# rbrito/deprecated-lame-mirror

Hardware: AMD Instinct MI355X
Metric: encoded audio seconds/sec (x real-time) at 44.1kHz stereo CBR128 (higher is better)
Workload: dtype f32

## Files before the change

### deprecated-lame-mirror_amd/csrc/lh_analysis.hip

```cpp
#include <stdint.h>
#include <math.h>

#ifdef LH_EMU
#include "hipemu.h"
#define LH_CONST static const
#else
#include <hip/hip_runtime.h>
#define LH_CONST __device__ static const
#endif

#if defined(LH_APROF) && !defined(LH_EMU)
__shared__ unsigned long long *lh_ap_base;
#define LH_PT(var) unsigned long long var = clock64()
#define LH_PA(idx, var) do { if (c.lane == 0) atomicAdd(&lh_ap_base[LH_NPROF * c.wave + 20 + (idx)], clock64() - var); } while (0)
#define LH_PC(idx) do { } while (0)
#endif
#define LH_CUSTOM_LDS "lh_lds_analysis.h"
#define LH_CUSTOM_SMP
#define LH_FZ_X(i) ((((i) >> 4) & 2) | (((i) >> 3) & 24) | (((i) >> 5) & 4))
#define LH_FZ(i) ((i) ^ LH_FZ_X(i))
#define LH_STAGE_IDX(i) LH_FZ(i)
#include "lh_static_tables.h"
#include "lh_dev_common.h"
#if !defined(LH_EMU)
#define LH_KRESTRICT __restrict__
#else
#define LH_KRESTRICT
#endif

#define LH_SPAN (lh_lds.work)
LH_DEVFN float
lh_smp(const LhCtx & c, int ch, int i)
{
    return LH_SPAN[ch * LH_BLKSIZE + LH_FZ(i)];
}

#include "lh_dev_psy_core.h"

struct LhGranuleAt {
    int     live;
    int     gr;
    long long at;
    long long frame_base;
};

LH_DEVFN LhGranuleAt
lh_granule_at(const LhStreamDesc & d, int g)
{
    LhGranuleAt o;
    int const nf = d.frame_end - d.frame_begin;
    int const fr = g / LH_NGR;
    o.live = g < LH_NGR * nf;
    o.gr = g - fr * LH_NGR;
    o.at = d.out_index + d.mid_rel + fr;
    o.frame_base = (long long) (576 * LH_NGR) * (d.frame_begin + fr) - LH_MF_START;
    return o;
}

LH_DEVFN LhStreamDesc
lh_desc_uniform(const LhStreamDesc * descs, int sidx)
{
    LhStreamDesc d = descs[sidx];
    d.pcm_l = lh_uni_ll(d.pcm_l);
    d.pcm_r = lh_uni_ll(d.pcm_r);
    d.pcm_base = lh_uni_ll(d.pcm_base);
    d.nsamples = lh_uni_ll(d.nsamples);
    d.out_index = lh_uni_ll(d.out_index);
    d.mid_rel = lh_uni_i(d.mid_rel);
    d.frame_begin = lh_uni_i(d.frame_begin);
    d.frame_end = lh_uni_i(d.frame_end);
    return d;
}

#ifdef LH_LSF
#define lh_attack_kernel lh_attack_kernel_lsf
#define lh_attack_scan_kernel lh_attack_scan_kernel_lsf
#define lh_analysis_kernel lh_analysis_kernel_lsf
#define lh_launch_analysis lh_launch_analysis_lsf
#define lh_emu_analysis lh_emu_analysis_lsf
#endif

#if defined(LH_APROF) && !defined(LH_EMU)
#define LH_AP_T0() unsigned long long ap_t = clock64()
#define LH_AP(k) do { unsigned long long const n_ = clock64(); if (c.lane == 0) atomicAdd(&aprof[64 * 0 + LH_NPROF * c.wave + (k)], n_ - ap_t); ap_t = n_; } while (0)
#else
#define LH_AP_T0() do { } while (0)
#define LH_AP(k) do { } while (0)
#endif
#define LH_FIR_SPAN 640

#ifndef LH_EMU
extern "C" __global__ void __launch_bounds__(64)
#else
void
#endif
lh_attack_kernel(const LhConfig * LH_KRESTRICT cfg, const int16_t * LH_KRESTRICT pcm, const float *pcmf, const LhStreamDesc * descs, LhMidFrame * frames,
                 int nstreams)
{
    __shared__ float span[2 * LH_FIR_SPAN];
    int const sidx = (int) blockIdx.y;
    LhCtx   c;
    c.cfg = cfg;
    c.T = nullptr;
    c.st = nullptr;
    c.pcm = pcm;
    c.pcmf = pcmf;
    c.d = lh_desc_uniform(descs, sidx);
    c.tid = (int) threadIdx.x;
    c.lane = c.tid;
    c.wave = 0;
    LhGranuleAt const ga = lh_granule_at(c.d, (int) blockIdx.x);
    if (!ga.live)
        return;
    int const lane = c.lane;
    int const n_chn_psy = (cfg->mode == LH_MODE_JOINT_STEREO) ? 4 : cfg->channels;
    int const bufbase = 576 + ga.gr * 576 - LH_FFTOFFSET;
    int const firbase = bufbase + 576 - 350 - LH_NSFIRLEN + 192;
    LhMidGr *mg = &frames[ga.at].small.gr[ga.gr];
    lh_stage_span < LH_FIR_SPAN, 64, 1 > (c, span, span + LH_FIR_SPAN, ga.frame_base + firbase);
    LH_WAVE_SYNC();
    {
        int const i0 = 9 * lane;
        float   x[2][30], y[2][9];
#pragma unroll
        for (int ch = 0; ch < 2; ch++)
#pragma unroll
            for (int t = 0; t < 30; t++)
                x[ch][t] = span[ch * LH_FIR_SPAN + i0 + t];
#pragma unroll
        for (int ch = 0; ch < 2; ch++)
#pragma unroll
            for (int m = 0; m < 9; m++) {
                float   sum1 = x[ch][m + 10], sum2 = 0.0;
#pragma unroll
                for (int j = 0; j < ((LH_NSFIRLEN - 1) / 2) - 1; j += 2) {
                    sum1 += lh_hp_fir[j] * (x[ch][m + j] + x[ch][m + LH_NSFIRLEN - j]);
                    sum2 += lh_hp_fir[j + 1] * (x[ch][m + j + 1] + x[ch][m + LH_NSFIRLEN - j - 1]);
                }
                y[ch][m] = sum1 + sum2;
            }
        LH_WAVE_SYNC();
#pragma unroll
        for (int ch = 0; ch < 2; ch++)
#pragma unroll
            for (int m = 0; m < 9; m++)
                span[ch * LH_FIR_SPAN + i0 + m] = y[ch][m];
    }
    LH_WAVE_SYNC();
    float   fl[9], fr[9];
#pragma unroll
    for (int k = 0; k < 9; k++) {
        fl[k] = span[lane + 64 * k];
        fr[k] = span[LH_FIR_SPAN + lane + 64 * k];
    }
    for (int chn = 0; chn < n_chn_psy; chn++) {
        uint32_t pk[8], pk8 = 0;
#pragma unroll
        for (int k = 0; k < 9; k++) {
            float const l = fl[k], r = fr[k];
            float const v = (chn == 0) ? l : (chn == 1) ? r : (chn == 2) ? l + r : l - r;
            if (k < 8)
                pk[k] = lh_f32_as_u32(lh_fabsf(v));
            else
                pk8 = lh_f32_as_u32(lh_fabsf(v));
        }
        {
            uint32_t const m8 = lh_wave_max8(pk);
            uint32_t const m9 = lh_wave_max_u32(pk8);
            if (lane < 9)
                mg->peak[chn][lane] = lh_u32_as_f32(lane == 8 ? m9 : m8);
        }
    }
}

#ifndef LH_SCAN_BLOCK
#define LH_SCAN_BLOCK 4
#endif
#ifndef LH_EMU
extern "C" __global__ void __launch_bounds__(64)
#else
void
#endif
lh_attack_scan_kernel(const LhConfig * LH_KRESTRICT cfg, const LhTables * LH_KRESTRICT T, const LhStreamDesc * descs, const LhStreamState * states,
                      LhMidFrame * frames, int nstreams)
{
    int const sidx = (int) blockIdx.x;
    int const lane = (int) threadIdx.x;
    LhStreamDesc const d = lh_desc_uniform(descs, sidx);
    int const nf = d.frame_end - d.frame_begin;
    if (nf <= 0)
        return;
    const LhStreamState *st = &states[sidx];
    int const n_chn_psy = lh_uni_i((cfg->mode == LH_MODE_JOINT_STEREO) ? 4 : cfg->channels);
    int const channels = lh_uni_i(cfg->channels), short_blocks = lh_uni_i(cfg->short_blocks);
    int const chn = lane >> 4, i = lane & 15, grp = lane & 48;
    int const mine = chn < n_chn_psy;
    float   le = st->last_en_subshort[chn][i < 9 ? i : 0];
    int     last_att = st->last_attacks[chn];
    float const thresh = T->attack_threshold[chn];
    int     bt_old0 = lh_uni_i(st->blocktype_old[0]), bt_old1 = lh_uni_i(st->blocktype_old[1]);
    int const ng = LH_NGR * nf;
    float   pk_blk[LH_SCAN_BLOCK];
#pragma unroll
    for (int j = 0; j < LH_SCAN_BLOCK; j++) {
        int const g = (j < ng) ? j : 0;
        pk_blk[j] = frames[d.out_index + d.mid_rel + g / LH_NGR].small.gr[g % LH_NGR].peak[chn][i < 9 ? i : 0];
    }
    for (int g0 = 0; g0 < ng; g0 += LH_SCAN_BLOCK) {
        float   pk_cur[LH_SCAN_BLOCK], ssf_blk[LH_SCAN_BLOCK];
        int     nsa_blk[LH_SCAN_BLOCK][4];
#pragma unroll
        for (int j = 0; j < LH_SCAN_BLOCK; j++) {
            int const gn = g0 + LH_SCAN_BLOCK + j, g = (gn < ng) ? gn : 0;
            pk_cur[j] = pk_blk[j];
            pk_blk[j] = frames[d.out_index + d.mid_rel + g / LH_NGR].small.gr[g % LH_NGR].peak[chn][i < 9 ? i : 0];
        }
#pragma unroll
        for (int j = 0; j < LH_SCAN_BLOCK; j++) {
            float const pk = pk_cur[j];
            float const fresh = pk < 1.0f ? 1.0f : pk;
            float const old = lh_shfl_f32(le, grp + ((i + 6) & 15)), older = lh_shfl_f32(le, grp + ((i + 4) & 15));
            float const got = lh_shfl_f32(fresh, grp + ((i - 3) & 15));
            float const e = (i < 3) ? old : got;
            float const e1 = lh_shfl_f32(e, grp + ((i - 1) & 15)), e0 = lh_shfl_f32(e, grp + ((i - 2) & 15));
            float const then = (i < 3) ? older : e0;
            float const ai = (i < 3) ? e / then : (e > then) ? e / then : (then > e * 10.0f) ? then / (e * 10.0f) : 0.0f;
            float const whole = e0 + e1 + e;
            int const tail_low = e * 6 < whole, mid_low = e1 * 6 < whole;
            uint64_t const over_all = lh_ballot(i < 12 && ai > thresh);
            unsigned const over = (unsigned) (over_all >> (16 * chn)) & 0xfffu;
            float   en_short[4];
            en_short[0] = lh_shfl_f32(whole, grp + 2);
            en_short[1] = lh_shfl_f32(whole, grp + 5);
            en_short[2] = lh_shfl_f32(whole, grp + 8);
            en_short[3] = lh_shfl_f32(whole, grp + 11);
            ssf_blk[j] = tail_low ? (mid_low ? 0.25f : 0.5f) : 1.0f;
            int    *nsa = nsa_blk[j];
            le = fresh;
            for (int gq = 0; gq < 4; gq++) {
                unsigned const bits = (over >> (3 * gq)) & 7u;
                nsa[gq] = bits ? ((bits & 1u) ? 1 : (bits & 2u) ? 2 : 3) : 0;
            }
            for (int q = 1; q < 4; q++) {
                float const u = en_short[q - 1];
                float const v = en_short[q];
                float const m = (u > v) ? u : v;
                if (m < 40000) {
                    if (u < 1.7f * v && v < 1.7f * u) {
                        if (q == 1 && nsa[0] <= nsa[q])
                            nsa[0] = 0;
                        nsa[q] = 0;
                    }
                }
            }
        }
#pragma unroll
        for (int j = 0; j < LH_SCAN_BLOCK; j++) {
            int const g = g0 + j;
            if (g >= ng)
                break;
            int const fr = g / LH_NGR, gr = g - fr * LH_NGR;
            LhMidGr *mg = &frames[d.out_index + d.mid_rel + fr].small.gr[gr];
            int    *nsa = nsa_blk[j];
            float const ssf = ssf_blk[j];
            int     uselong = 1;
            if (nsa[0] <= last_att)
                nsa[0] = 0;
            if (last_att == 3 || nsa[0] + nsa[1] + nsa[2] + nsa[3]) {
                uselong = 0;
                if (nsa[1] && nsa[0])
                    nsa[1] = 0;
                if (nsa[2] && nsa[1])
                    nsa[2] = 0;
                if (nsa[3] && nsa[2])
                    nsa[3] = 0;
            }
            if (!mine) {
                nsa[0] = nsa[1] = nsa[2] = nsa[3] = 0;
                uselong = 1;
            }
            else
                last_att = nsa[2];
            if (i == 5 || i == 8 || i == 11)
                mg->sub_short_factor[chn][(i - 5) / 3] = mine ? ssf : 1.0f;
            if (i < 4)
                mg->ns_attacks[chn][i] = (int8_t) (i == 0 ? nsa[0] : i == 1 ? nsa[1] : i == 2 ? nsa[2] : nsa[3]);
            {
                uint64_t const shorts = lh_ballot(!uselong);
                int const s0 = (int) (shorts & 1u), s1 = (int) ((shorts >> 16) & 1u), s23 = (int) ((shorts >> 32) & 0x10001u) != 0;
                int     ul0 = !s0, ul1 = (channels == 2) ? !s1 : 1;
                int     btd[2];
                if (s23)
                    ul0 = ul1 = 0;
                if (short_blocks == 1 && !(ul0 && ul1))
                    ul0 = ul1 = 0;
                if (short_blocks == 2)
                    ul0 = ul1 = 1;
                if (short_blocks == 3)
                    ul0 = ul1 = 0;
                for (int ch = 0; ch < 2; ch++) {
                    int     blocktype = LH_NORM_TYPE;
                    int     was = ch ? bt_old1 : bt_old0;
                    if (ch ? ul1 : ul0) {
                        if (was == LH_SHORT_TYPE)
                            blocktype = LH_STOP_TYPE;
                    }
                    else {
                        blocktype = LH_SHORT_TYPE;
                        if (was == LH_NORM_TYPE)
                            was = LH_START_TYPE;
                        if (was == LH_STOP_TYPE)
                            was = LH_SHORT_TYPE;
                    }
                    btd[ch] = was;
                    if (ch)
                        bt_old1 = lh_uni_i(blocktype);
                    else
                        bt_old0 = lh_uni_i(blocktype);
                }
                if (lane < 2) {
                    mg->uselong[lane] = (int8_t) (lane ? ul1 : ul0);
                    mg->block_type[lane] = (int8_t) (lane ? btd[1] : btd[0]);
                }
            }
        }
    }
}

template < int K1 > LH_DEVFN void
lh_fht_unit_fz(lh_f32x4 tw, float *fz, int u)
{
    constexpr int kx = K1 >> 1, k2 = K1 << 1, k3 = k2 + K1, k4 = k2 << 1;
    int const blk = u / kx, i = u - blk * kx;
    int const axis = (i == 0);
    int const lo = blk * k4 + i;
    int const hi = blk * k4 + (axis ? kx : K1 - i);
    int     al[4], ah[4];
    if (K1 == 4) {
        int const x = LH_FZ_X(lo);
#pragma unroll
        for (int j = 0; j < 4; j++) {
            al[j] = (lo + j * K1) ^ x;
            ah[j] = (hi + j * K1) ^ x;
        }
    }
    else if (K1 == 16) {
        int const x = LH_FZ_X(blk * k4);
#pragma unroll
        for (int j = 0; j < 4; j++) {
            al[j] = (lo + j * K1) ^ x ^ (j >= 2 ? 2 : 0);
            ah[j] = (hi + j * K1) ^ x ^ (j >= 2 ? 2 : 0);
        }
    }
    else if (K1 == 64) {
#pragma unroll
        for (int j = 0; j < 4; j++) {
            al[j] = (lo + j * K1) ^ LH_FZ_X(64 * j);
            ah[j] = (hi + j * K1) ^ (2 ^ LH_FZ_X(64 * j));
        }
    }
    else {
        int const xl = LH_FZ_X(lo), xh = LH_FZ_X(hi);
#pragma unroll
        for (int j = 0; j < 4; j++) {
            al[j] = (lo + j * K1) ^ xl;
            ah[j] = (hi + j * K1) ^ xh;
        }
    }
    float const p0 = fz[al[0]], p1 = fz[al[1]], p2 = fz[al[2]], p3 = fz[al[3]];
    float const q0 = fz[ah[0]], q1 = fz[ah[1]], q2 = fz[ah[2]], q3 = fz[ah[3]];
    float const s01 = p0 + p1, d01 = p0 - p1, s23 = p2 + p3, d23 = p2 - p3;
    float const r2 = (float) (LH_SQRT2 * q2), r3 = (float) (LH_SQRT2 * q3);
    float const t01 = q0 + q1, u01 = q0 - q1;
    float const a_l0 = s01 + s23, a_l1 = d01 + d23, a_l2 = s01 - s23, a_l3 = d01 - d23;
    float const a_h0 = t01 + r2, a_h1 = u01 + r3, a_h2 = t01 - r2, a_h3 = u01 - r3;
    LhRot const rq1 = lh_rot(tw.z, tw.w, p1, q1);
    LhRot const rq3 = lh_rot(tw.z, tw.w, p3, q3);
    float const le = p0 + rq1.along, lm = p0 - rq1.along;
    float const he = q0 + rq1.across, hm = q0 - rq1.across;
    float const l2e = p2 + rq3.along, l2m = p2 - rq3.along;
    float const h2e = q2 + rq3.across, h2m = q2 - rq3.across;
    LhRot const ra = lh_rot(tw.x, tw.y, l2e, h2m);
    LhRot const rb = lh_rot(tw.y, tw.x, h2e, l2m);
    fz[al[0]] = axis ? a_l0 : le + ra.along;
    fz[al[1]] = axis ? a_l1 : lm + rb.across;
    fz[al[2]] = axis ? a_l2 : le - ra.along;
    fz[al[3]] = axis ? a_l3 : lm - rb.across;
    fz[ah[0]] = axis ? a_h0 : he + rb.along;
    fz[ah[1]] = axis ? a_h1 : hm + ra.across;
    fz[ah[2]] = axis ? a_h2 : he - rb.along;
    fz[ah[3]] = axis ? a_h3 : hm - ra.across;
}

LH_DEVFN void
lh_fft_long_inplace(const LhCtx & c, float *x)
{
    const float *w = c.T->fft_window;
    int const lane = c.lane;
    float   o[2][8];
#pragma unroll
    for (int q = 0; q < 2; q++) {
        int const jj = lane + 64 * q;
        int const i = (int) lh_rev8((unsigned) jj);
        const float *xs = x + (i ^ LH_FZ_X(i));
        float   f0, f1, f2, f3, ww;
        f0 = w[i] * xs[0];
        ww = w[i + 0x200] * xs[0x200];
        f1 = f0 - ww;
        f0 = f0 + ww;
        f2 = w[i + 0x100] * xs[0x100];
        ww = w[i + 0x300] * xs[0x300];
        f3 = f2 - ww;
        f2 = f2 + ww;
        o[q][0] = f0 + f2;
        o[q][2] = f0 - f2;
        o[q][1] = f1 + f3;
        o[q][3] = f1 - f3;
        f0 = w[i + 0x001] * xs[0x001];
        ww = w[i + 0x201] * xs[0x201];
        f1 = f0 - ww;
        f0 = f0 + ww;
        f2 = w[i + 0x101] * xs[0x101];
        ww = w[i + 0x301] * xs[0x301];
        f3 = f2 - ww;
        f2 = f2 + ww;
        o[q][4] = f0 + f2;
        o[q][6] = f0 - f2;
        o[q][5] = f1 + f3;
        o[q][7] = f1 - f3;
    }
    {
        lh_f32x4 tw[4][2];
#pragma unroll
        for (int stage = 0; stage < 4; stage++) {
            int const kx = 2 << (2 * stage);
#pragma unroll
            for (int q = 0; q < 2; q++)
                tw[stage][q] = *(const lh_f32x4 *) c.T->fht_tw[stage][(lane + 64 * q) % kx];
        }
        LH_WAVE_SYNC_MEM();
#pragma unroll
        for (int q = 0; q < 2; q++) {
            int const at = 4 * (lane + 64 * q), xa = LH_FZ_X(at);
#pragma unroll
            for (int k = 0; k < 4; k++) {
                x[(at + k) ^ xa] = o[q][k];
                x[(at + k + LH_BLKSIZE / 2) ^ xa] = o[q][4 + k];
            }
        }
        LH_WAVE_SYNC_MEM();
#pragma unroll
        for (int q = 0; q < 2; q++)
            lh_fht_unit_fz < 4 > (tw[0][q], x, lane + 64 * q);
        LH_WAVE_SYNC_MEM();
#pragma unroll
        for (int q = 0; q < 2; q++)
            lh_fht_unit_fz < 16 > (tw[1][q], x, lane + 64 * q);
        LH_WAVE_SYNC_MEM();
#pragma unroll
        for (int q = 0; q < 2; q++)
            lh_fht_unit_fz < 64 > (tw[2][q], x, lane + 64 * q);
        LH_WAVE_SYNC_MEM();
#pragma unroll
        for (int q = 0; q < 2; q++)
            lh_fht_unit_fz < 256 > (tw[3][q], x, lane + 64 * q);
        LH_WAVE_SYNC_MEM();
    }
}

LH_DEVFN void
lh_fft_short_inplace(const LhCtx & c, float *x)
{
    const float *ws = c.T->fft_window_s;
    int const lane = c.lane;
    float   o[2][8];
#pragma unroll
    for (int q = 0; q < 2; q++) {
        int const t = lane + 64 * q, tt = t < 3 * (LH_BLKSIZE_S / 8) ? t : 0;
        int const b = tt >> 5, j = tt & 31;
        int const k = (576 / 3) * (b + 1);
        int const i = (int) lh_rev8((unsigned) (j << 2));
        float   f0, f1, f2, f3, w;
        f0 = ws[i] * x[LH_FZ(i + k)];
        w = ws[0x7f - i] * x[LH_FZ(i + k + 0x80)];
        f1 = f0 - w;
        f0 = f0 + w;
        f2 = ws[i + 0x40] * x[LH_FZ(i + k + 0x40)];
        w = ws[0x3f - i] * x[LH_FZ(i + k + 0xc0)];
        f3 = f2 - w;
        f2 = f2 + w;
        o[q][0] = f0 + f2;
        o[q][2] = f0 - f2;
        o[q][1] = f1 + f3;
        o[q][3] = f1 - f3;
        f0 = ws[i + 0x01] * x[LH_FZ(i + k + 0x01)];
        w = ws[0x7e - i] * x[LH_FZ(i + k + 0x81)];
        f1 = f0 - w;
        f0 = f0 + w;
        f2 = ws[i + 0x41] * x[LH_FZ(i + k + 0x41)];
        w = ws[0x3e - i] * x[LH_FZ(i + k + 0xc1)];
        f3 = f2 - w;
        f2 = f2 + w;
        o[q][4] = f0 + f2;
        o[q][6] = f0 - f2;
        o[q][5] = f1 + f3;
        o[q][7] = f1 - f3;
    }
    LH_WAVE_SYNC_MEM();
#pragma unroll
    for (int q = 0; q < 2; q++) {
        int const t = lane + 64 * q;
        if (t < 3 * (LH_BLKSIZE_S / 8)) {
            int const at = (t >> 5) * LH_BLKSIZE_S + 4 * (t & 31);
#pragma unroll
            for (int k = 0; k < 4; k++) {
                x[LH_FZ(at + k)] = o[q][k];
                x[LH_FZ(at + k + LH_BLKSIZE_S / 2)] = o[q][4 + k];
            }
        }
    }
    LH_WAVE_SYNC_MEM();
    for (int t = lane; t < 3 * (LH_BLKSIZE_S / 8); t += 64) {
        int const b = t >> 5, u = t & 31;
        lh_fht_unit_fz < 4 > (*(const lh_f32x4 *) c.T->fht_tw[0][u % 2], x + b * LH_BLKSIZE_S, u);
    }
    LH_WAVE_SYNC_MEM();
    for (int t = lane; t < 3 * (LH_BLKSIZE_S / 8); t += 64) {
        int const b = t >> 5, u = t & 31;
        lh_fht_unit_fz < 16 > (*(const lh_f32x4 *) c.T->fht_tw[1][u % 8], x + b * LH_BLKSIZE_S, u);
    }
    LH_WAVE_SYNC_MEM();
    for (int t = lane; t < 3 * (LH_BLKSIZE_S / 8); t += 64) {
        int const b = t >> 5, u = t & 31;
        lh_fht_unit_fz < 64 > (*(const lh_f32x4 *) c.T->fht_tw[2][u % 32], x + b * LH_BLKSIZE_S, u);
    }
    LH_WAVE_SYNC_MEM();
}

LH_DEVFN void
lh_an_spectra_short(const LhCtx & c, int w, int both, const float *wl, const float *wr, int first, float *out_own, float *out_ms)
{
    float const sqrt2_half = (float) (LH_SQRT2 * 0.5f);
    int const n = LH_BLKSIZE_S, h = n >> 1;
    for (int m = c.lane; m <= h; m += 64) {
        int const ire = first + m, iim = first + ((m == 0) ? 0 : (n - m));
        float const lre = wl[LH_FZ(ire)], lim = wl[LH_FZ(iim)], rre = wr[LH_FZ(ire)], rim = wr[LH_FZ(iim)];
        float const ore = w ? rre : lre, oim = w ? rim : lim;
        float const mre = (w ? lre - rre : lre + rre) * sqrt2_half, mim = (w ? lim - rim : lim + rim) * sqrt2_half;
        out_own[m] = (m == 0) ? ore * ore : (ore * ore + oim * oim) * 0.5f;
        if (both)
            out_ms[m] = (m == 0) ? mre * mre : (mre * mre + mim * mim) * 0.5f;
    }
}

LH_DEVFN void
lh_an_spectra(const LhCtx & c, int w, int own, int ms, float *work)
{
    float const sqrt2_half = (float) (LH_SQRT2 * 0.5f);
    const float *wl = work, *wr = work + LH_BLKSIZE;
    float   eo[9], em[9];
#pragma unroll
    for (int k = 0; k < 9; k++) {
        int const m0 = c.lane + 64 * k, m = m0 <= LH_BLKSIZE / 2 ? m0 : LH_BLKSIZE / 2;
        int const ire = m, iim = (m == 0) ? 0 : (LH_BLKSIZE - m);
        float const lre = wl[LH_FZ(ire)], lim = wl[LH_FZ(iim)], rre = wr[LH_FZ(ire)], rim = wr[LH_FZ(iim)];
        float const ore = w ? rre : lre, oim = w ? rim : lim;
        float const mre = (w ? lre - rre : lre + rre) * sqrt2_half, mim = (w ? lim - rim : lim + rim) * sqrt2_half;
        eo[k] = (m == 0) ? ore * ore : (ore * ore + oim * oim) * 0.5f;
        em[k] = (m == 0) ? mre * mre : (mre * mre + mim * mim) * 0.5f;
    }
    LH_SYNC_WG_LDS();
#pragma unroll
    for (int k = 0; k < 9; k++) {
        int const m = c.lane + 64 * k;
        if (m <= LH_BLKSIZE / 2) {
            if (own)
                work[w * LH_AN_ROW + m] = eo[k];
            if (ms)
                work[(w + 2) * LH_AN_ROW + m] = em[k];
        }
    }
}

#ifndef LH_EMU
extern "C" __global__ void __launch_bounds__(LH_NT, 6)
#else
void
#endif
lh_analysis_kernel(const LhConfig * LH_KRESTRICT cfg, const LhTables * LH_KRESTRICT T, const int16_t * LH_KRESTRICT pcm, const float *pcmf, const LhStreamDesc * descs,
                   LhMidFrame * frames, int nstreams, LhStreamState * states)
{
#if defined(LH_APROF) && !defined(LH_EMU)
    unsigned long long *aprof = &states[blockIdx.y].prof[0][0];
    if (threadIdx.x == 0)
        lh_ap_base = aprof;
#endif
    LH_AP_T0();
    LhLds & L = lh_lds;
    LhLds & P = L;
    float  *const work = L.work;
#define LH_AN_E(chn) (work + (chn) * LH_AN_ROW)
    int const sidx = (int) blockIdx.y;
    LhCtx   c;
    c.cfg = cfg;
    c.T = T;
    c.st = nullptr;
    c.pcm = pcm;
    c.pcmf = pcmf;
    c.d = lh_desc_uniform(descs, sidx);
    c.tid = (int) threadIdx.x;
    c.lane = c.tid & 63;
    c.wave = lh_uni_i(c.tid >> 6);
    LhGranuleAt const ga = lh_granule_at(c.d, (int) blockIdx.x);
    if (!ga.live)
        return;
    int const lane = c.lane, w = c.wave, gr = ga.gr;
    int const n_chn_psy = (cfg->mode == LH_MODE_JOINT_STEREO) ? 4 : cfg->channels;
    int const bufbase = 576 + gr * 576 - LH_FFTOFFSET;
    LhMidGr *mg = &frames[ga.at].small.gr[gr];
    if (c.tid < 2)
        L.uselong[c.tid] = mg->uselong[c.tid];
    LH_AP(0);
    lh_stage_span < LH_BLKSIZE, LH_NT > (c, LH_SPAN, LH_SPAN + LH_BLKSIZE, ga.frame_base + bufbase);
    LH_SYNC_WG_LDS();
    LH_AP(1);
// ... 159 lines not shown
```

### deprecated-lame-mirror_amd/csrc/lh_dev_common.h

```cpp
#ifndef LH_DEV_COMMON_H
#define LH_DEV_COMMON_H

#include <stdint.h>
#include "lamehip_types.h"
#include "lh_device.h"
#include "lh_wave.h"
#include "lh_dev_math.h"

#define LH_NT 128
#ifdef LH_LSF
#define LH_NGR 1
#define LH_IS_LSF 1
#define LH_RATE8K(c) ((c).rate8k)
#else
#define LH_NGR 2
#define LH_IS_LSF 0
#define LH_RATE8K(c) 0
#endif
#define LH_BLOCK LH_NT
#define LH_SQRT2 1.41421356237309504880

#ifdef LH_EMU
#define LH_SYNC_WG() do { __syncthreads(); } while (0)
#define LH_SYNC_WG_LDS() do { __syncthreads(); } while (0)
// ... 443 lines not shown
    const LhTables *T;
    LhStreamState *st;
    const int16_t *pcm;
    const float *pcmf;
    LhStreamDesc d;
    long long frame_base;
    int     lane, wave, tid;
    int     ns, ns_amp, sfb21_extra, full_outer_loop, subblock_gain;
    int     rate8k;
    int     l21;
};

LH_DEVFN void
lh_ctx_hot(LhCtx & c)
{
    c.ns = lh_uni_i(c.cfg->noise_shaping);
    c.ns_amp = lh_uni_i(c.cfg->noise_shaping_amp);
    c.sfb21_extra = lh_uni_i(c.cfg->sfb21_extra);
    c.full_outer_loop = lh_uni_i(c.cfg->full_outer_loop);
    c.subblock_gain = lh_uni_i(c.cfg->subblock_gain);
    c.l21 = lh_uni_i(c.T->sfb_l[LH_SBPSY_L]);
#ifdef LH_LSF
    c.rate8k = lh_uni_i(c.cfg->samplerate <= 8000);
#else
    c.rate8k = 0;
#endif
}

#ifdef LH_DEBUG_DUMP
#define LH_ROUTE(c, k) do { if ((c).lane == 0) (c).st->dbg_route[(c).wave][k] += 1u; } while (0)
#else
#define LH_ROUTE(c, k) do { } while (0)
#endif
#define LH_ROUTE_ZERO(bt) ((bt) == LH_NORM_TYPE ? LH_RT_ZERO_norm : (bt) == LH_SHORT_TYPE ? LH_RT_ZERO_short : LH_RT_ZERO_other)

#ifdef LH_EMU
#define LH_AS_GLOBAL(type, p) (p)
#else
template < typename X > __device__ __forceinline__ X *
lh_as_global(X * p)
{
    typedef __attribute__((address_space(1))) X GX;
    unsigned long long const u = (unsigned long long) p;
    unsigned lo = (unsigned) __builtin_amdgcn_readfirstlane((int) (unsigned) u);
    unsigned hi = (unsigned) __builtin_amdgcn_readfirstlane((int) (unsigned) (u >> 32));
    asm volatile("" : "+s"(lo), "+s"(hi));
    return (X *) (GX *) (((unsigned long long) hi << 32) | lo);
}
#define LH_AS_GLOBAL(type, p) lh_as_global < type > (p)
#endif
LH_DEVFN LhCtx
lh_ctx_load(void)
{
    LhCtx   o;
    o.cfg = LH_AS_GLOBAL(const LhConfig, lh_lds.ctx.cfg);
    o.T = LH_AS_GLOBAL(const LhTables, lh_lds.ctx.T);
    o.st = LH_AS_GLOBAL(LhStreamState, lh_lds.ctx.st);
    o.pcm = LH_AS_GLOBAL(const int16_t, lh_lds.ctx.pcm);
    o.pcmf = LH_AS_GLOBAL(const float, lh_lds.ctx.pcmf);
    o.d = lh_lds.ctx.d;
    o.frame_base = lh_lds.ctx.frame_base;
    o.tid = (int) threadIdx.x;
    o.lane = o.tid & 63;
    o.wave = lh_uni_i(o.tid >> 6);
    lh_ctx_hot(o);
    return o;
}

LH_DEVFN int
lh_cfg_class(const LhCtx & c)
{
    int const ok = !LH_IS_LSF && (c.ns == 1 || c.ns == 2) && c.ns_amp == 1 && c.full_outer_loop == 0 && c.sfb21_extra == 0
        && c.l21 <= 418;
    return ok ? c.ns : 0;
}

LH_DEVFN int
lh_granule_is_usual(const LhCtx & c, int block_type, int substep)
{
    return (block_type == LH_NORM_TYPE && (substep & 2) == 0) ? lh_cfg_class(c) : 0;
}

LH_DEVFN int
lh_granule_is_usual_short(const LhCtx & c, int block_type, int substep)
{
    return (block_type == LH_SHORT_TYPE && (substep & 2) == 0 && c.subblock_gain == 1) ? lh_cfg_class(c) : 0;
}

LH_DEVFN void
lh_pin_usual(LhCtx & c, int nsh)
{
    if (nsh)
        c.ns = nsh;
    c.ns_amp = 1;
    c.full_outer_loop = 0;
    c.sfb21_extra = 0;
    c.rate8k = 0;
    if (c.l21 > 418)
        __builtin_unreachable();
}

LH_DEVFN void
lh_pin_usual(LhQR & R)
{
    R.block_type = LH_NORM_TYPE;
    R.sfb_lmax = LH_SBPSY_L;
    R.sfb_smin = LH_SBPSY_S;
    R.psy_lmax = LH_SBPSY_L;
    R.psymax = LH_SBPSY_L;
    R.sfbmax = LH_SBPSY_L;
    R.sfbdivide = 11;
    if ((R.substep_shaping & 2) != 0)
        __builtin_unreachable();
}

LH_DEVFN void
lh_pin_usual_short(LhQR & R)
{
    R.block_type = LH_SHORT_TYPE;
    R.sfb_lmax = 0;
    R.sfb_smin = 0;
    R.psy_lmax = 0;
    R.psymax = 3 * LH_SBPSY_S;
    R.sfbmax = 3 * LH_SBPSY_S;
    R.sfbdivide = 3 * LH_SBPSY_S - 18;
    if ((R.substep_shaping & 2) != 0)
        __builtin_unreachable();
}

LH_DEVFN void
lh_rg_put(const LhCtx & c, const LhQR & R, const LhGrR & g)
{
    if (c.lane == 0) {
        lh_lds.rg[c.wave].R = R;
        lh_lds.rg[c.wave].g = g;
    }
    LH_WAVE_SYNC();
}

LH_DEVFN void
lh_stage_window(const LhCtx & c, float (*mf)[LH_MF_NEEDED], long long base)
{
    float const scale = c.cfg->pcm_scale;
    long long const last = c.d.nsamples - 1;
    float const mix = c.cfg->pcm_mix;
    float const scale_r = c.cfg->pcm_scale_r;
    if (c.pcmf) {
        for (int t = c.tid; t < 2 * LH_MF_NEEDED; t += LH_NT) {
            int const ch = t >= LH_MF_NEEDED, i = t - ch * LH_MF_NEEDED;
            long long const p = base + i;
            float   v = 0.0f;
            if (p >= 0 && p <= last && p >= c.d.pcm_base)
                v = c.pcmf[(ch == 0 ? c.d.pcm_l : c.d.pcm_r) + (p - c.d.pcm_base)];
            mf[ch][i] = v;
        }
        return;
    }
    if (mix != 0.0f) {
        for (int i = c.tid; i < LH_MF_NEEDED; i += LH_NT) {
            long long const p = base + i;
            float   v = 0.0f;
            if (p >= 0 && p <= last && p >= c.d.pcm_base) {
                float const xl = (float) c.pcm[c.d.pcm_l + (p - c.d.pcm_base)];
                float const xr = (float) c.pcm[c.d.pcm_r + (p - c.d.pcm_base)];
                v = xl * scale + xr * mix;
            }
            mf[0][i] = v;
            mf[1][i] = 0.0f;
        }
        return;
    }
    {
        long long const lo = base, hi = base + LH_MF_NEEDED - 1;
        long long const ol = c.d.pcm_l + (base - c.d.pcm_base), orr = c.d.pcm_r + (base - c.d.pcm_base);
        int const inside = lo >= 0 && lo >= c.d.pcm_base && hi <= last && ((ol | orr) & 1) == 0;
        if (lh_uni_i(inside)) {
            const uint32_t *pl = (const uint32_t *) (c.pcm + ol), *pr = (const uint32_t *) (c.pcm + orr);
            uint32_t v[16];
#pragma unroll
            for (int u = 0; u < 8; u++) {
                int const j = c.tid + LH_NT * u;
                int const jj = j < LH_MF_NEEDED / 2 ? j : LH_MF_NEEDED / 2 - 1;
                v[u] = pl[jj];
                v[8 + u] = pr[jj];
            }
#pragma unroll
            for (int u = 0; u < 8; u++) {
                int const j = c.tid + LH_NT * u;
                if (j < LH_MF_NEEDED / 2) {
                    lh_f32x2 a, b;
                    a.x = (float) (int16_t) (v[u] & 0xffffu) * scale;
                    a.y = (float) (int16_t) (v[u] >> 16) * scale;
                    b.x = (float) (int16_t) (v[8 + u] & 0xffffu) * scale_r;
                    b.y = (float) (int16_t) (v[8 + u] >> 16) * scale_r;
                    ((lh_f32x2 *) mf[0])[j] = a;
                    ((lh_f32x2 *) mf[1])[j] = b;
                }
            }
            return;
        }
    }
    for (int t0 = c.tid; t0 < 2 * LH_MF_NEEDED; t0 += 6 * LH_NT) {
        int16_t v[6];
#pragma unroll
        for (int u = 0; u < 6; u++) {
            int const t = t0 + u * LH_NT;
            int const tt = t < 2 * LH_MF_NEEDED ? t : 2 * LH_MF_NEEDED - 1;
            int const ch = tt >= LH_MF_NEEDED, i = tt - ch * LH_MF_NEEDED;
            long long p = base + i;
            p = p < 0 ? 0 : (p > last ? last : p);
            p = p < c.d.pcm_base ? c.d.pcm_base : p;
            v[u] = (c.d.nsamples > 0) ? c.pcm[(ch == 0 ? c.d.pcm_l : c.d.pcm_r) + (p - c.d.pcm_base)] : (int16_t) 0;
        }
#pragma unroll
        for (int u = 0; u < 6; u++) {
            int const t = t0 + u * LH_NT;
            if (t < 2 * LH_MF_NEEDED) {
                int const ch = t >= LH_MF_NEEDED, i = t - ch * LH_MF_NEEDED;
                long long const p = base + i;
                mf[ch][i] = (p < 0 || p > last) ? 0.0f : (float) v[u] * (ch == 0 ? scale : scale_r);
            }
        }
    }
}

#ifndef LH_STAGE_IDX
#define LH_STAGE_IDX(i) (i)
#endif
template < int N, int NT, int PLAIN = 0 > LH_DEVFN void
lh_stage_span(const LhCtx & c, float *d0, float *d1, long long base)
{
#define LH_STAGE_AT(i) (PLAIN ? (i) : LH_STAGE_IDX(i))
    float const scale = c.cfg->pcm_scale;
    long long const last = c.d.nsamples - 1;
    float const mix = c.cfg->pcm_mix;
    float const scale_r = c.cfg->pcm_scale_r;
    if (c.pcmf) {
        for (int t = c.tid; t < 2 * N; t += NT) {
            int const ch = t >= N, i = t - ch * N;
            long long const p = base + i;
            float   v = 0.0f;
            if (p >= 0 && p <= last && p >= c.d.pcm_base)
                v = c.pcmf[(ch == 0 ? c.d.pcm_l : c.d.pcm_r) + (p - c.d.pcm_base)];
            (ch ? d1 : d0)[LH_STAGE_AT(i)] = v;
        }
        return;
    }
    if (mix != 0.0f) {
        for (int i = c.tid; i < N; i += NT) {
            long long const p = base + i;
            float   v = 0.0f;
            if (p >= 0 && p <= last && p >= c.d.pcm_base) {
                float const xl = (float) c.pcm[c.d.pcm_l + (p - c.d.pcm_base)];
                float const xr = (float) c.pcm[c.d.pcm_r + (p - c.d.pcm_base)];
                v = xl * scale + xr * mix;
            }
            d0[LH_STAGE_AT(i)] = v;
            d1[LH_STAGE_AT(i)] = 0.0f;
        }
        return;
    }
    {
        long long const lo = base, hi = base + N - 1;
        long long const ol = c.d.pcm_l + (base - c.d.pcm_base), orr = c.d.pcm_r + (base - c.d.pcm_base);
        int const inside = lo >= 0 && lo >= c.d.pcm_base && hi <= last && ((ol | orr) & 1) == 0;
        static_assert(N % 2 == 0, "pairs");
        constexpr int U = (N / 2 + NT - 1) / NT;
        if (lh_uni_i(inside)) {
            const uint32_t *pl = (const uint32_t *) (c.pcm + ol), *pr = (const uint32_t *) (c.pcm + orr);
            uint32_t v[2 * U];
#pragma unroll
            for (int u = 0; u < U; u++) {
                int const j = c.tid + NT * u;
                int const jj = j < N / 2 ? j : N / 2 - 1;
                v[u] = pl[jj];
                v[U + u] = pr[jj];
            }
#pragma unroll
            for (int u = 0; u < U; u++) {
                int const j = c.tid + NT * u;
                if (j < N / 2) {
                    lh_f32x2 a, b;
                    a.x = (float) (int16_t) (v[u] & 0xffffu) * scale;
                    a.y = (float) (int16_t) (v[u] >> 16) * scale;
                    b.x = (float) (int16_t) (v[U + u] & 0xffffu) * scale_r;
                    b.y = (float) (int16_t) (v[U + u] >> 16) * scale_r;
                    *(lh_f32x2 *) &d0[LH_STAGE_AT(2 * j)] = a;
                    *(lh_f32x2 *) &d1[LH_STAGE_AT(2 * j)] = b;
                }
            }
            return;
        }
    }
    for (int t = c.tid; t < 2 * N; t += NT) {
        int const ch = t >= N, i = t - ch * N;
        long long const p0 = base + i;
        long long p = p0 < 0 ? 0 : (p0 > last ? last : p0);
        int16_t v;
        p = p < c.d.pcm_base ? c.d.pcm_base : p;
        v = (c.d.nsamples > 0) ? c.pcm[(ch == 0 ? c.d.pcm_l : c.d.pcm_r) + (p - c.d.pcm_base)] : (int16_t) 0;
        (ch ? d1 : d0)[LH_STAGE_AT(i)] = (p0 < 0 || p0 > last) ? 0.0f : (float) v * (ch == 0 ? scale : scale_r);
    }
}
#undef LH_STAGE_AT

#ifndef LH_CUSTOM_SMP
LH_DEVFN float
lh_smp(const LhCtx & c, int ch, int i)
{
    return lh_lds.mf[ch][i];
}
#endif

#endif
```

### deprecated-lame-mirror_amd/csrc/lh_subband.hip

```cpp
#include <stdint.h>
#include <math.h>

#ifdef LH_EMU
#include "hipemu.h"
#define LH_CONST static const
#else
#include <hip/hip_runtime.h>
#define LH_CONST __device__ static const
#endif

#define LH_CUSTOM_LDS "lh_lds_subband.h"
#define LH_MF_SWZ(i) ((i) ^ (((i) >> 1) & 16))
#define LH_STAGE_IDX(i) LH_MF_SWZ(i)
#define LH_SB_STRIDE 33
#define LH_ENW_TAPS (lh_lds.enw)
#define LH_MDCT_WIN (lh_lds.mwin)
#define LH_MF_PADDED ((LH_MF_NEEDED + 63) / 64 * 64)
#include "lh_static_tables.h"
#include "lh_dev_common.h"
#if !defined(LH_EMU)
#define LH_KRESTRICT __restrict__
#else
#define LH_KRESTRICT
#endif

#include "lh_dev_mdct.h"

#if defined(LH_APROF) && !defined(LH_EMU)
#define LH_AP_T0() unsigned long long ap_t = clock64()
#define LH_AP(k) do { unsigned long long const n_ = clock64(); if (c.lane == 0) atomicAdd(&c.st->prof[c.wave][(k)], n_ - ap_t); ap_t = n_; } while (0)
#else
#define LH_AP_T0() do { } while (0)
#define LH_AP(k) do { } while (0)
#endif
#define LH_SB_CARRY ((LH_SB_GRANULE + 63) / 64)
#ifndef LH_SB_RUN
#define LH_SB_RUN 16
#endif

#ifdef LH_LSF
#define lh_subband_kernel lh_subband_kernel_lsf
#define lh_launch_subband lh_launch_subband_lsf
#define lh_emu_subband lh_emu_subband_lsf
#endif

#ifndef LH_EMU
extern "C" __global__ void __launch_bounds__(LH_NT, 2)
#else
void
#endif
lh_subband_kernel(const LhConfig * LH_KRESTRICT cfg, const LhTables * LH_KRESTRICT T, const int16_t * LH_KRESTRICT pcm, const float *pcmf, const LhStreamDesc * descs,
                  LhStreamState * states, LhMidFrame * frames, int nstreams)
{
    LhLds & L = lh_lds;
    int const sidx = (int) blockIdx.y;
    constexpr int ngr = LH_NGR, fs = 576 * LH_NGR;
    LhCtx   c;
    c.cfg = cfg;
    c.T = T;
    c.st = &states[sidx];
    c.pcm = pcm;
    c.pcmf = pcmf;
    c.d = descs[sidx];
    c.d.pcm_l = lh_uni_ll(c.d.pcm_l);
    c.d.pcm_r = lh_uni_ll(c.d.pcm_r);
    c.d.pcm_base = lh_uni_ll(c.d.pcm_base);
    c.d.nsamples = lh_uni_ll(c.d.nsamples);
    c.d.out_index = lh_uni_ll(c.d.out_index);
    c.d.mid_rel = lh_uni_i(c.d.mid_rel);
    c.d.frame_begin = lh_uni_i(c.d.frame_begin);
    c.d.frame_end = lh_uni_i(c.d.frame_end);
    c.tid = (int) threadIdx.x;
    c.lane = c.tid & 63;
    c.wave = lh_uni_i(c.tid >> 6);
    lh_ctx_hot(c);
    int const f0 = c.d.frame_begin + LH_SB_RUN * (int) blockIdx.x;
    int const f1 = (f0 + LH_SB_RUN < c.d.frame_end) ? f0 + LH_SB_RUN : c.d.frame_end;
    if (f0 >= c.d.frame_end)
        return;
    int const w = c.wave, lane = c.lane, tid = c.tid;
    if (tid == 0) {
        L.ctx.cfg = c.cfg;
        L.ctx.T = c.T;
        L.ctx.st = c.st;
        L.ctx.pcm = c.pcm;
        L.ctx.pcmf = c.pcmf;
        L.ctx.bytes = nullptr;
        L.ctx.d = c.d;
        L.ctx.frame_base = 0;
    }
    float   sb[LH_SB_CARRY];
    LH_AP_T0();
    for (int i = tid; i < 288; i += LH_NT)
        L.enw[i] = lh_enwindow[i < 285 ? i : 284];
    for (int i = tid; i < 4 * 36; i += LH_NT)
        L.mwin[i] = lh_mdct_win[i];
    lh_stage_span < LH_MF_NEEDED, LH_NT > (c, L.mf[0], L.mf[1], (long long) fs * f0 - LH_MF_START - fs);
    LH_SYNC_WG_LDS();
    lh_polyphase(w);
#pragma unroll
    for (int k = 0; k < LH_SB_CARRY; k++)
        sb[k] = L.u.mdct.sb[w][ngr][(lane + 64 * k < LH_SB_GRANULE) ? lane + 64 * k : 0];
    LH_SYNC_WG_LDS();
    LH_AP(8);
    for (int f = f0; f < f1; f++) {
        long long const at = c.d.out_index + c.d.mid_rel + (f - c.d.frame_begin);
        lh_stage_span < LH_MF_NEEDED, LH_NT > (c, L.mf[0], L.mf[1], (long long) fs * f - LH_MF_START);
        if (tid < 4) {
            int const gr = tid >> 1, ch = tid & 1;
            L.block_type[gr][ch] = (gr < ngr) ? (int) frames[at].small.gr[gr].block_type[ch] : LH_NORM_TYPE;
        }
#pragma unroll
        for (int k = 0; k < LH_SB_CARRY; k++)
            if (lane + 64 * k < LH_SB_GRANULE)
                L.u.mdct.sb[w][0][lane + 64 * k] = sb[k];
        LH_SYNC_WG_LDS();
        LH_AP(9);
        lh_polyphase(w);
        LH_SYNC_WG_LDS();
        LH_AP(10);
        lh_mdct_granules(w);
#pragma unroll
        for (int k = 0; k < LH_SB_CARRY; k++)
            sb[k] = L.u.mdct.sb[w][ngr][(lane + 64 * k < LH_SB_GRANULE) ? lane + 64 * k : 0];
        LH_SYNC_WG_LDS();
        LH_AP(11);
        {
            lh_f32x4 *dst = (lh_f32x4 *) frames[at].xr.xr;
            const lh_f32x4 *src = (const lh_f32x4 *) L.xr;
            for (int i = tid; i < 576; i += LH_NT)
                dst[i] = src[i];
        }
        LH_SYNC_WG_LDS();
        LH_AP(12);
    }
    if (f1 == c.d.frame_end) {
#pragma unroll
        for (int k = 0; k < LH_SB_CARRY; k++) {
            int const i = lane + 64 * k, slot = i / LH_SB_STRIDE, col = i - slot * LH_SB_STRIDE;
            if (i < LH_SB_GRANULE && col < 32)
                c.st->sb_prev[w][slot * 32 + col] = sb[k];
        }
    }
}

#ifndef LH_EMU
extern "C" int
lh_launch_subband(const LhConfig * cfg, const LhTables * T, const int16_t * pcm, const float *pcmf, const LhStreamDesc * descs,
                  LhStreamState * states, LhMidPools mid, int nstreams, int max_frames, void *stream)
{
    if (nstreams <= 0 || max_frames <= 0)
        return 0;
    hipLaunchKernelGGL(lh_subband_kernel, dim3((unsigned) ((max_frames + LH_SB_RUN - 1) / LH_SB_RUN), (unsigned) nstreams),
                       dim3(LH_NT), 0, (hipStream_t) stream, cfg, T, pcm, pcmf, descs, states, mid.frames, nstreams);
    return (int) hipGetLastError();
}
#else
extern "C" int
lh_emu_subband(const LhConfig * cfg, const LhTables * T, const int16_t * pcm, const float *pcmf, const LhStreamDesc * descs,
               LhStreamState * states, const LhMidPools * pools, int nstreams, int max_frames)
{
    LhMidPools const mid = *pools;
    hipemu_dim3 grid = { (unsigned) ((max_frames + LH_SB_RUN - 1) / LH_SB_RUN), (unsigned) nstreams, 1 }, block = { LH_NT, 1, 1 };
    hipemu_run(grid, block,[=] () {
               lh_subband_kernel(cfg, T, pcm, pcmf, descs, states, mid.frames, nstreams);
               }
    );
    return 0;
}
#endif
```

Before: 84400.

## Prefetch next-frame PCM and block types in subband loop; deepen attack-scan prefetch

The subband kernel now issues the global PCM loads and block-type reads for the next frame into registers before running the current frame's polyphase. It then writes them to LDS at the top of the next iteration, so memory latency overlaps with compute. The attack-scan kernel keeps a multi-block queue of peak values, prefetching LH_SCAN_DEPTH blocks ahead instead of one. The cost is more register pressure, plus a fast path that applies only to aligned int16 input without pcm mixing, falling back to the old staging otherwise.

```diff
diff --git a/deprecated-lame-mirror_amd/csrc/lh_analysis.hip b/deprecated-lame-mirror_amd/csrc/lh_analysis.hip
--- a/deprecated-lame-mirror_amd/csrc/lh_analysis.hip
+++ b/deprecated-lame-mirror_amd/csrc/lh_analysis.hip
@@ -176,6 +176,9 @@
 #ifndef LH_SCAN_BLOCK
 #define LH_SCAN_BLOCK 4
 #endif
+#ifndef LH_SCAN_DEPTH
+#define LH_SCAN_DEPTH 4
+#endif
 #ifndef LH_EMU
 extern "C" __global__ void __launch_bounds__(64)
 #else
@@ -200,127 +203,135 @@
     float const thresh = T->attack_threshold[chn];
     int     bt_old0 = lh_uni_i(st->blocktype_old[0]), bt_old1 = lh_uni_i(st->blocktype_old[1]);
     int const ng = LH_NGR * nf;
-    float   pk_blk[LH_SCAN_BLOCK];
-#pragma unroll
-    for (int j = 0; j < LH_SCAN_BLOCK; j++) {
-        int const g = (j < ng) ? j : 0;
-        pk_blk[j] = frames[d.out_index + d.mid_rel + g / LH_NGR].small.gr[g % LH_NGR].peak[chn][i < 9 ? i : 0];
-    }
-    for (int g0 = 0; g0 < ng; g0 += LH_SCAN_BLOCK) {
-        float   pk_cur[LH_SCAN_BLOCK], ssf_blk[LH_SCAN_BLOCK];
-        int     nsa_blk[LH_SCAN_BLOCK][4];
+    float   pk_q[LH_SCAN_DEPTH][LH_SCAN_BLOCK];
+#pragma unroll
+    for (int dq = 0; dq < LH_SCAN_DEPTH; dq++)
 #pragma unroll
         for (int j = 0; j < LH_SCAN_BLOCK; j++) {
-            int const gn = g0 + LH_SCAN_BLOCK + j, g = (gn < ng) ? gn : 0;
-            pk_cur[j] = pk_blk[j];
-            pk_blk[j] = frames[d.out_index + d.mid_rel + g / LH_NGR].small.gr[g % LH_NGR].peak[chn][i < 9 ? i : 0];
-        }
-#pragma unroll
-        for (int j = 0; j < LH_SCAN_BLOCK; j++) {
-            float const pk = pk_cur[j];
-            float const fresh = pk < 1.0f ? 1.0f : pk;
-            float const old = lh_shfl_f32(le, grp + ((i + 6) & 15)), older = lh_shfl_f32(le, grp + ((i + 4) & 15));
-            float const got = lh_shfl_f32(fresh, grp + ((i - 3) & 15));
-            float const e = (i < 3) ? old : got;
-            float const e1 = lh_shfl_f32(e, grp + ((i - 1) & 15)), e0 = lh_shfl_f32(e, grp + ((i - 2) & 15));
-            float const then = (i < 3) ? older : e0;
-            float const ai = (i < 3) ? e / then : (e > then) ? e / then : (then > e * 10.0f) ? then / (e * 10.0f) : 0.0f;
-            float const whole = e0 + e1 + e;
-            int const tail_low = e * 6 < whole, mid_low = e1 * 6 < whole;
-            uint64_t const over_all = lh_ballot(i < 12 && ai > thresh);
-            unsigned const over = (unsigned) (over_all >> (16 * chn)) & 0xfffu;
-            float   en_short[4];
-            en_short[0] = lh_shfl_f32(whole, grp + 2);
-            en_short[1] = lh_shfl_f32(whole, grp + 5);
-            en_short[2] = lh_shfl_f32(whole, grp + 8);
-            en_short[3] = lh_shfl_f32(whole, grp + 11);
-            ssf_blk[j] = tail_low ? (mid_low ? 0.25f : 0.5f) : 1.0f;
-            int    *nsa = nsa_blk[j];
-            le = fresh;
-            for (int gq = 0; gq < 4; gq++) {
-                unsigned const bits = (over >> (3 * gq)) & 7u;
-                nsa[gq] = bits ? ((bits & 1u) ? 1 : (bits & 2u) ? 2 : 3) : 0;
-            }
-            for (int q = 1; q < 4; q++) {
-                float const u = en_short[q - 1];
-                float const v = en_short[q];
-                float const m = (u > v) ? u : v;
-                if (m < 40000) {
-                    if (u < 1.7f * v && v < 1.7f * u) {
-                        if (q == 1 && nsa[0] <= nsa[q])
-                            nsa[0] = 0;
-                        nsa[q] = 0;
+            int const gn = LH_SCAN_BLOCK * dq + j, g = (gn < ng) ? gn : 0;
+            pk_q[dq][j] = frames[d.out_index + d.mid_rel + g / LH_NGR].small.gr[g % LH_NGR].peak[chn][i < 9 ? i : 0];
+        }
+    for (int gs = 0; gs < ng; gs += LH_SCAN_DEPTH * LH_SCAN_BLOCK) {
+#pragma unroll
+        for (int dq = 0; dq < LH_SCAN_DEPTH; dq++) {
+            int const g0 = gs + LH_SCAN_BLOCK * dq;
+            if (g0 >= ng)
+                break;
+            float   pk_cur[LH_SCAN_BLOCK], ssf_blk[LH_SCAN_BLOCK];
+            int     nsa_blk[LH_SCAN_BLOCK][4];
+#pragma unroll
+            for (int j = 0; j < LH_SCAN_BLOCK; j++) {
+                int const gn = g0 + LH_SCAN_DEPTH * LH_SCAN_BLOCK + j, g = (gn < ng) ? gn : 0;
+                pk_cur[j] = pk_q[dq][j];
+                pk_q[dq][j] = frames[d.out_index + d.mid_rel + g / LH_NGR].small.gr[g % LH_NGR].peak[chn][i < 9 ? i : 0];
+            }
+#pragma unroll
+            for (int j = 0; j < LH_SCAN_BLOCK; j++) {
+                float const pk = pk_cur[j];
+                float const fresh = pk < 1.0f ? 1.0f : pk;
+                float const old = lh_shfl_f32(le, grp + ((i + 6) & 15)), older = lh_shfl_f32(le, grp + ((i + 4) & 15));
+                float const got = lh_shfl_f32(fresh, grp + ((i - 3) & 15));
+                float const e = (i < 3) ? old : got;
+                float const e1 = lh_shfl_f32(e, grp + ((i - 1) & 15)), e0 = lh_shfl_f32(e, grp + ((i - 2) & 15));
+                float const then = (i < 3) ? older : e0;
+                float const ai = (i < 3) ? e / then : (e > then) ? e / then : (then > e * 10.0f) ? then / (e * 10.0f) : 0.0f;
+                float const whole = e0 + e1 + e;
+                int const tail_low = e * 6 < whole, mid_low = e1 * 6 < whole;
+                uint64_t const over_all = lh_ballot(i < 12 && ai > thresh);
+                unsigned const over = (unsigned) (over_all >> (16 * chn)) & 0xfffu;
+                float   en_short[4];
+                en_short[0] = lh_shfl_f32(whole, grp + 2);
+                en_short[1] = lh_shfl_f32(whole, grp + 5);
+                en_short[2] = lh_shfl_f32(whole, grp + 8);
+                en_short[3] = lh_shfl_f32(whole, grp + 11);
+                ssf_blk[j] = tail_low ? (mid_low ? 0.25f : 0.5f) : 1.0f;
+                int    *nsa = nsa_blk[j];
+                le = fresh;
+                for (int gq = 0; gq < 4; gq++) {
+                    unsigned const bits = (over >> (3 * gq)) & 7u;
+                    nsa[gq] = bits ? ((bits & 1u) ? 1 : (bits & 2u) ? 2 : 3) : 0;
+                }
+                for (int q = 1; q < 4; q++) {
+                    float const u = en_short[q - 1];
+                    float const v = en_short[q];
+                    float const m = (u > v) ? u : v;
+                    if (m < 40000) {
+                        if (u < 1.7f * v && v < 1.7f * u) {
+                            if (q == 1 && nsa[0] <= nsa[q])
+                                nsa[0] = 0;
+                            nsa[q] = 0;
+                        }
                     }
                 }
             }
-        }
-#pragma unroll
-        for (int j = 0; j < LH_SCAN_BLOCK; j++) {
-            int const g = g0 + j;
-            if (g >= ng)
-                break;
-            int const fr = g / LH_NGR, gr = g - fr * LH_NGR;
-            LhMidGr *mg = &frames[d.out_index + d.mid_rel + fr].small.gr[gr];
-            int    *nsa = nsa_blk[j];
-            float const ssf = ssf_blk[j];
-            int     uselong = 1;
-            if (nsa[0] <= last_att)
-                nsa[0] = 0;
-            if (last_att == 3 || nsa[0] + nsa[1] + nsa[2] + nsa[3]) {
-                uselong = 0;
-                if (nsa[1] && nsa[0])
-                    nsa[1] = 0;
-                if (nsa[2] && nsa[1])
-                    nsa[2] = 0;
-                if (nsa[3] && nsa[2])
-                    nsa[3] = 0;
-            }
-            if (!mine) {
-                nsa[0] = nsa[1] = nsa[2] = nsa[3] = 0;
-                uselong = 1;
-            }
-            else
-                last_att = nsa[2];
-            if (i == 5 || i == 8 || i == 11)
-                mg->sub_short_factor[chn][(i - 5) / 3] = mine ? ssf : 1.0f;
-            if (i < 4)
-                mg->ns_attacks[chn][i] = (int8_t) (i == 0 ? nsa[0] : i == 1 ? nsa[1] : i == 2 ? nsa[2] : nsa[3]);
-            {
-                uint64_t const shorts = lh_ballot(!uselong);
-                int const s0 = (int) (shorts & 1u), s1 = (int) ((shorts >> 16) & 1u), s23 = (int) ((shorts >> 32) & 0x10001u) != 0;
-                int     ul0 = !s0, ul1 = (channels == 2) ? !s1 : 1;
-                int     btd[2];
-                if (s23)
-                    ul0 = ul1 = 0;
-                if (short_blocks == 1 && !(ul0 && ul1))
-                    ul0 = ul1 = 0;
-                if (short_blocks == 2)
-                    ul0 = ul1 = 1;
-                if (short_blocks == 3)
-                    ul0 = ul1 = 0;
-                for (int ch = 0; ch < 2; ch++) {
-                    int     blocktype = LH_NORM_TYPE;
-                    int     was = ch ? bt_old1 : bt_old0;
-                    if (ch ? ul1 : ul0) {
-                        if (was == LH_SHORT_TYPE)
-                            blocktype = LH_STOP_TYPE;
+#pragma unroll
+            for (int j = 0; j < LH_SCAN_BLOCK; j++) {
+                int const g = g0 + j;
+                if (g >= ng)
+                    break;
+                int const fr = g / LH_NGR, gr = g - fr * LH_NGR;
+                LhMidGr *mg = &frames[d.out_index + d.mid_rel + fr].small.gr[gr];
+                int    *nsa = nsa_blk[j];
+                float const ssf = ssf_blk[j];
+                int     uselong = 1;
+                if (nsa[0] <= last_att)
+                    nsa[0] = 0;
+                if (last_att == 3 || nsa[0] + nsa[1] + nsa[2] + nsa[3]) {
+                    uselong = 0;
+                    if (nsa[1] && nsa[0])
+                        nsa[1] = 0;
+                    if (nsa[2] && nsa[1])
+                        nsa[2] = 0;
+                    if (nsa[3] && nsa[2])
+                        nsa[3] = 0;
+                }
+                if (!mine) {
+                    nsa[0] = nsa[1] = nsa[2] = nsa[3] = 0;
+                    uselong = 1;
+                }
+                else
+                    last_att = nsa[2];
+                if (i == 5 || i == 8 || i == 11)
+                    mg->sub_short_factor[chn][(i - 5) / 3] = mine ? ssf : 1.0f;
+                if (i < 4)
+                    mg->ns_attacks[chn][i] = (int8_t) (i == 0 ? nsa[0] : i == 1 ? nsa[1] : i == 2 ? nsa[2] : nsa[3]);
+                {
+                    uint64_t const shorts = lh_ballot(!uselong);
+                    int const s0 = (int) (shorts & 1u), s1 = (int) ((shorts >> 16) & 1u), s23 = (int) ((shorts >> 32) & 0x10001u) != 0;
+                    int     ul0 = !s0, ul1 = (channels == 2) ? !s1 : 1;
+                    int     btd[2];
+                    if (s23)
+                        ul0 = ul1 = 0;
+                    if (short_blocks == 1 && !(ul0 && ul1))
+                        ul0 = ul1 = 0;
+                    if (short_blocks == 2)
+                        ul0 = ul1 = 1;
+                    if (short_blocks == 3)
+                        ul0 = ul1 = 0;
+                    for (int ch = 0; ch < 2; ch++) {
+                        int     blocktype = LH_NORM_TYPE;
+                        int     was = ch ? bt_old1 : bt_old0;
+                        if (ch ? ul1 : ul0) {
+                            if (was == LH_SHORT_TYPE)
+                                blocktype = LH_STOP_TYPE;
+                        }
+                        else {
+                            blocktype = LH_SHORT_TYPE;
+                            if (was == LH_NORM_TYPE)
+                                was = LH_START_TYPE;
+                            if (was == LH_STOP_TYPE)
+                                was = LH_SHORT_TYPE;
+                        }
+                        btd[ch] = was;
+                        if (ch)
+                            bt_old1 = lh_uni_i(blocktype);
+                        else
+                            bt_old0 = lh_uni_i(blocktype);
                     }
-                    else {
-                        blocktype = LH_SHORT_TYPE;
-                        if (was == LH_NORM_TYPE)
-                            was = LH_START_TYPE;
-                        if (was == LH_STOP_TYPE)
-                            was = LH_SHORT_TYPE;
+                    if (lane < 2) {
+                        mg->uselong[lane] = (int8_t) (lane ? ul1 : ul0);
+                        mg->block_type[lane] = (int8_t) (lane ? btd[1] : btd[0]);
                     }
-                    btd[ch] = was;
-                    if (ch)
-                        bt_old1 = lh_uni_i(blocktype);
-                    else
-                        bt_old0 = lh_uni_i(blocktype);
-                }
-                if (lane < 2) {
-                    mg->uselong[lane] = (int8_t) (lane ? ul1 : ul0);
-                    mg->block_type[lane] = (int8_t) (lane ? btd[1] : btd[0]);
                 }
             }
         }
diff --git a/deprecated-lame-mirror_amd/csrc/lh_dev_common.h b/deprecated-lame-mirror_amd/csrc/lh_dev_common.h
--- a/deprecated-lame-mirror_amd/csrc/lh_dev_common.h
+++ b/deprecated-lame-mirror_amd/csrc/lh_dev_common.h
@@ -769,6 +769,67 @@
         (ch ? d1 : d0)[LH_STAGE_AT(i)] = (p0 < 0 || p0 > last) ? 0.0f : (float) v * (ch == 0 ? scale : scale_r);
     }
 }
+
+template < int N, int NT > struct LhSpanAhead {
+    uint32_t v[2 * ((N / 2 + NT - 1) / NT)];
+    int     ahead;
+    int     usual;
+    float   scale, scale_r;
+};
+
+template < int N, int NT > LH_DEVFN void
+lh_span_begin(const LhCtx & c, LhSpanAhead < N, NT > &r)
+{
+    r.ahead = 0;
+    r.usual = lh_uni_i(!c.pcmf && c.cfg->pcm_mix == 0.0f);
+    r.scale = c.cfg->pcm_scale;
+    r.scale_r = c.cfg->pcm_scale_r;
+}
+
+template < int N, int NT > LH_DEVFN void
+lh_span_fetch(const LhCtx & c, long long base, int live, LhSpanAhead < N, NT > &r)
+{
+    constexpr int U = (N / 2 + NT - 1) / NT;
+    long long const last = c.d.nsamples - 1;
+    long long const lo = base, hi = base + N - 1;
+    long long const ol = c.d.pcm_l + (base - c.d.pcm_base), orr = c.d.pcm_r + (base - c.d.pcm_base);
+    int const inside = live && r.usual && lo >= 0 && lo >= c.d.pcm_base && hi <= last && ((ol | orr) & 1) == 0;
+    r.ahead = lh_uni_i(inside);
+    if (r.ahead) {
+        const uint32_t *pl = (const uint32_t *) (c.pcm + ol), *pr = (const uint32_t *) (c.pcm + orr);
+#pragma unroll
+        for (int u = 0; u < U; u++) {
+            int const j = c.tid + NT * u;
+            int const jj = j < N / 2 ? j : N / 2 - 1;
+            r.v[u] = pl[jj];
+            r.v[U + u] = pr[jj];
+        }
+    }
+}
+
+template < int N, int NT, int PLAIN = 0 > LH_DEVFN void
+lh_span_put(const LhCtx & c, const LhSpanAhead < N, NT > &r, float *d0, float *d1, long long base)
+{
+    constexpr int U = (N / 2 + NT - 1) / NT;
+    if (!r.ahead) {
+        lh_stage_span < N, NT, PLAIN > (c, d0, d1, base);
+        return;
+    }
+    float const scale = r.scale, scale_r = r.scale_r;
+#pragma unroll
+    for (int u = 0; u < U; u++) {
+        int const j = c.tid + NT * u;
+        if (j < N / 2) {
+            lh_f32x2 a, b;
+            a.x = (float) (int16_t) (r.v[u] & 0xffffu) * scale;
+            a.y = (float) (int16_t) (r.v[u] >> 16) * scale;
+            b.x = (float) (int16_t) (r.v[U + u] & 0xffffu) * scale_r;
+            b.y = (float) (int16_t) (r.v[U + u] >> 16) * scale_r;
+            *(lh_f32x2 *) &d0[LH_STAGE_AT(2 * j)] = a;
+            *(lh_f32x2 *) &d1[LH_STAGE_AT(2 * j)] = b;
+        }
+    }
+}
 #undef LH_STAGE_AT
 
 #ifndef LH_CUSTOM_SMP
diff --git a/deprecated-lame-mirror_amd/csrc/lh_subband.hip b/deprecated-lame-mirror_amd/csrc/lh_subband.hip
--- a/deprecated-lame-mirror_amd/csrc/lh_subband.hip
+++ b/deprecated-lame-mirror_amd/csrc/lh_subband.hip
@@ -97,6 +97,13 @@
         L.mwin[i] = lh_mdct_win[i];
     lh_stage_span < LH_MF_NEEDED, LH_NT > (c, L.mf[0], L.mf[1], (long long) fs * f0 - LH_MF_START - fs);
     LH_SYNC_WG_LDS();
+    LhSpanAhead < LH_MF_NEEDED, LH_NT > win;
+    lh_span_begin < LH_MF_NEEDED, LH_NT > (c, win);
+    lh_span_fetch < LH_MF_NEEDED, LH_NT > (c, (long long) fs * f0 - LH_MF_START, 1, win);
+    int const bt_gr = (tid >> 1) & 1, bt_ch = tid & 1, bt_mine = tid < 4 && bt_gr < ngr;
+    int     bt_ahead = LH_NORM_TYPE;
+    if (bt_mine)
+        bt_ahead = (int) frames[c.d.out_index + c.d.mid_rel + (f0 - c.d.frame_begin)].small.gr[bt_gr].block_type[bt_ch];
     lh_polyphase(w);
 #pragma unroll
     for (int k = 0; k < LH_SB_CARRY; k++)
@@ -105,17 +112,18 @@
     LH_AP(8);
     for (int f = f0; f < f1; f++) {
         long long const at = c.d.out_index + c.d.mid_rel + (f - c.d.frame_begin);
-        lh_stage_span < LH_MF_NEEDED, LH_NT > (c, L.mf[0], L.mf[1], (long long) fs * f - LH_MF_START);
-        if (tid < 4) {
-            int const gr = tid >> 1, ch = tid & 1;
-            L.block_type[gr][ch] = (gr < ngr) ? (int) frames[at].small.gr[gr].block_type[ch] : LH_NORM_TYPE;
-        }
+        lh_span_put < LH_MF_NEEDED, LH_NT > (c, win, L.mf[0], L.mf[1], (long long) fs * f - LH_MF_START);
+        if (tid < 4)
+            L.block_type[bt_gr][bt_ch] = bt_ahead;
 #pragma unroll
         for (int k = 0; k < LH_SB_CARRY; k++)
             if (lane + 64 * k < LH_SB_GRANULE)
                 L.u.mdct.sb[w][0][lane + 64 * k] = sb[k];
         LH_SYNC_WG_LDS();
         LH_AP(9);
+        lh_span_fetch < LH_MF_NEEDED, LH_NT > (c, (long long) fs * (f + 1) - LH_MF_START, f + 1 < f1, win);
+        if (bt_mine && f + 1 < f1)
+            bt_ahead = (int) frames[at + 1].small.gr[bt_gr].block_type[bt_ch];
         lh_polyphase(w);
         LH_SYNC_WG_LDS();
         LH_AP(10);
```

New measurement: 84640, median of 6. About the same (+0.3%).
